# zhaihongjia/SplatLoc

Hardware: AMD Instinct MI355X
Metric: fwd+bwd frames/s @1080p, 500k Gaussians, 32 feat-ch; HBM GB/s vs roofline (higher is better)
Workload: dtype f32

## Files before the change

splatloc_amd/csrc/capi.hip:

```cpp
#include <string.h>

#include <mutex>
#include <unordered_map>
#include <string>
#include <vector>

#include "common.h"

namespace sr {

static thread_local std::string g_last_error;
static int g_deterministic = 0;
static int g_split_max_waves = SPLIT_MAX_WAVES;
void set_split_max_waves(int waves) { g_split_max_waves = waves < 0 ? SPLIT_MAX_WAVES : (waves > SPLIT_MAX_WAVES ? SPLIT_MAX_WAVES : waves); }
int split_max_waves() { return g_split_max_waves; }

void set_hip_error(hipError_t e, const char* what)
{
    g_last_error = std::string(what) + ": " + hipGetErrorString(e);
}

void set_error_text(const char* text) { g_last_error = text; }

struct StageRec { int stage; hipEvent_t a, b; };
// ... 129 lines not shown
    const size_t n = (size_t)(R > 0 ? R : 1);
    const size_t nv = (size_t)(V > 0 ? V : 1);
    const size_t tiles = (size_t)((W + TILE - 1) / TILE) * (size_t)((H + TILE - 1) / TILE) * nv;
    BinLayout L;
    size_t o = 0;
    auto take = [&](size_t bytes) { size_t at = o; o = align_up(o + bytes, 256); return at; };
    L.valsA = take(4 * n);
    L.keysA = take(4 * n);
    L.keysB = take(4 * n);
    L.valsB = take(4 * n);
    L.ranges = take(8 * (tiles > 0 ? tiles : 1));
    L.sort_tmp = take(sort_tmp_bytes((int64_t)n));
    L.irec = take(32 * n);
    L.ipack = take(4 * n);
    L.featp = take((C % 4) ? (size_t)(P > 0 ? P : 1) * padded_channels(C) * sizeof(float) : 16);
    L.gacc = take((size_t)(P > 0 ? P : 1) * nv * gacc_row_floats(C) * sizeof(float));
    L.pose_acc = take(POSE_ACC_BYTES);
    const bool ck = C <= 4 && 4 * (size_t)tiles <= (size_t)SPLIT_MAX_WAVES;
    L.ckpt = take(ck ? nv * (size_t)SPLIT_PARTS_MAX * (size_t)(C + 2) * (size_t)W * (size_t)H * sizeof(float) : 16);
    L.tile_order = take(4 * (tiles > 0 ? tiles : 1));
    L.nparts = take(4 * (tiles > 0 ? tiles : 1));
    L.bytes = o;
    return L;
}

BinView bin_view(void* base, int32_t P, int32_t V, int64_t R, int32_t W, int32_t H, int32_t C)
{
    const BinLayout L = bin_layout(P, V, R, W, H, C);
    char* b = reinterpret_cast<char*>(base);
    BinView v;
    v.point_list = reinterpret_cast<uint32_t*>(b + L.valsA);
// ... 17 lines not shown
{
    return align_up((size_t)W * H * 4 * (size_t)(V > 0 ? V : 1), 256);
}

ImgView img_view(void* base, int32_t W, int32_t H, int32_t V)
{
    char* b = reinterpret_cast<char*>(base);
    ImgView v;
    v.final_T = reinterpret_cast<float*>(b);
    v.n_contrib = reinterpret_cast<uint32_t*>(b + img_plane_bytes(W, H, V));
    return v;
}

static int check_row_index_range(int32_t P, int32_t V, int32_t C)
{
    const uint64_t row = (uint64_t)(gacc_row_floats(C) > padded_channels(C) ? gacc_row_floats(C) : padded_channels(C));
    const uint64_t n = (uint64_t)P * (uint64_t)V;
    if (n > (1ull << 24) || n * row >= (1ull << 32)) return SPLATRASTER_ERR_UNSUPPORTED;
    return SPLATRASTER_OK;
}

static int check_settings(const splatraster_settings* s)
{
    if (!s) return SPLATRASTER_ERR_BAD_ARG;
    if (s->image_width <= 0 || s->image_height <= 0 || s->channels <= 0) return SPLATRASTER_ERR_BAD_ARG;
    if (s->bg_channels < 0) return SPLATRASTER_ERR_BAD_ARG;
    return SPLATRASTER_OK;
}

}

using namespace sr;

// ... 358 lines not shown
        if (gcv != 0 && gcv < C) grads.gc = gcv;
    }
    for (int v = 0; v < V; ++v) {
        const int gcv = views[v].color_grad_channels ? views[v].color_grad_channels : C;
        if (gcv != grads.gc) return SPLATRASTER_ERR_BAD_ARG;
        grads.dL_dlast[v] = grads.gc < C ? views[v].dL_dout_last : nullptr;
    }
    for (int v = 0; v < V; ++v) {
        grads.out_color[v] = views[v].out_color;
        grads.out_depth[v] = views[v].out_depth;
        grads.dL_dcolor[v] = views[v].dL_dout_color;
        grads.dL_ddepth[v] = views[v].dL_dout_depth;
        grads.dL_dalpha[v] = views[v].dL_dout_alpha;
        grads.dL_dmeans2D[v] = views[v].dL_dmeans2D;
    }
    const size_t gacc_n = (size_t)gacc_row_floats(C) * (size_t)P * (size_t)V;
    const bool det = g_deterministic != 0;
    long long* gacc64 = nullptr;
    if (det) {
        SR_HIP_CHECK(hipMallocAsync(reinterpret_cast<void**>(&gacc64), sizeof(long long) * gacc_n, stream));
        SR_HIP_CHECK(hipMemsetAsync(gacc64, 0, sizeof(long long) * gacc_n, stream));
    }
    const bool pose = dL_dviewmatrix && dL_dprojmatrix;
    const size_t fill = pose ? (size_t)(reinterpret_cast<char*>(b.pose_acc) - reinterpret_cast<char*>(b.gacc)) + POSE_ACC_BYTES
                             : sizeof(float) * gacc_n;
    SR_HIP_CHECK(hipMemsetAsync(b.gacc, 0, fill, stream));
    grads.bg = bg;
    grads.bg_channels = bg ? s->bg_channels : 0;
    {
        StageTimer t(SPLATRASTER_STAGE_COMPOSITE_BWD, stream);
        if (det) st = launch_composite_bwd(*s, P, V, R, g, b, im, (C % 4) ? b.featp : feat, C, grads, b.gacc, gacc64, 0, stream);
        if (!st) st = launch_composite_bwd(*s, P, V, R, g, b, im, (C % 4) ? b.featp : feat, C, grads, b.gacc, gacc64, 1, stream);
    }
    if (det) {
        if (!st) st = launch_fixed_to_float((int64_t)gacc_n, gacc64, b.gacc, stream);
        (void)hipFreeAsync(gacc64, stream);
    }
    if (st) return st;
    StageTimer t(SPLATRASTER_STAGE_PREPROCESS_BWD, stream);
    return launch_preprocess_bwd(*s, P, V, cams, grads, means3D, shs, scales, rotations, cov3D_precomp, g.clamped, g.rec,
                                 b.gacc, C, shs ? nullptr : dL_dcolors, dL_dmeans3D, dL_dopacities,
                                 cov3D_precomp ? nullptr : dL_dscales, cov3D_precomp ? nullptr : dL_drotations,
                                 cov3D_precomp ? dL_dcov3D : nullptr, dL_dshs, dL_dviewmatrix, dL_dprojmatrix, dL_dcampos,
                                 b.pose_acc, stream, raw);
}

}

extern "C" {

// ... 542 lines not shown
```

splatloc_amd/csrc/common.h:

```cpp
#pragma once
#include <hip/hip_runtime.h>
#include <stdint.h>

#include "../../include/splatraster.h"

namespace sr {

constexpr int TILE = SPLATRASTER_TILE;
constexpr int TILE_PIX = TILE * TILE;
constexpr float NEAR_Z = 0.2f;
constexpr float DILATION = 0.3f;
constexpr float ALPHA_MAX = 0.99f;
constexpr float ALPHA_MIN = 1.0f / 255.0f;
constexpr float T_EPS = 0.0001f;
constexpr int WAVE = 64;
constexpr int PREPROCESS_BLOCK = 256;
static inline int preprocess_blocks(int32_t P) { return (P + PREPROCESS_BLOCK - 1) / PREPROCESS_BLOCK; }

void set_hip_error(hipError_t e, const char* what);
void set_error_text(const char* text);

int lookback_error_init();
int lookback_error_poll();
int lookback_set_spin_limit(uint32_t limit);
// ... 172 lines not shown
size_t bin_scratch_bytes(int32_t P, int32_t V, int tiles);
bool use_bins(int32_t P, int32_t V, int gx, int gy , size_t scratch_bytes);
int launch_bin_count(const splatraster_settings& s, int32_t P, int32_t V, const GeomView& g, uint32_t* table, void* scan_tmp,
                     hipStream_t stream);
int launch_bin_scatter_sort(const splatraster_settings& s, int32_t P, int32_t V, int64_t R, const GeomView& g,
                            const uint32_t* table, const BinView& b, uint64_t* keys, hipStream_t stream);

int launch_emit(const splatraster_settings& s, int32_t P, int32_t V, int64_t R, const GeomView& g, uint32_t* keys,
                uint32_t* vals, uint32_t* ranges, uint32_t nranges, hipStream_t stream);
int launch_ranges_clear(int32_t tiles, uint32_t* ranges, hipStream_t stream);
int launch_payload(const splatraster_settings& s, int32_t V, int64_t R, const GeomView& g, const BinView& b, hipStream_t stream);
int launch_pad_features(int32_t P, int C, const float* feat, float* featp, hipStream_t stream);
static inline int padded_channels(int C) { return (C + 3) & ~3; }
constexpr int POSE_SETS = 16, POSE_SET_FLOATS = 64;
constexpr size_t POSE_ACC_BYTES = (size_t)POSE_SETS * POSE_SET_FLOATS * sizeof(float) + 256;
__host__ __device__ static inline int gacc_moment_offset(int C) { return ((C & 15) + 7 <= 16) ? C : ((C + 15) & ~15); }
__host__ __device__ static inline int gacc_row_floats(int C) { return (gacc_moment_offset(C) + 7 + 15) & ~15; }
#ifndef SR_SPLIT_MAX_WAVES
#define SR_SPLIT_MAX_WAVES 6144
#endif
constexpr int SPLIT_MAX_WAVES = SR_SPLIT_MAX_WAVES;
constexpr int SPLIT_MIN_LIST = 256;
#ifndef SR_SPLIT_PARTS
#define SR_SPLIT_PARTS 4
#endif
constexpr int SPLIT_PARTS = SR_SPLIT_PARTS;
constexpr int SPLIT_PARTS_MAX = 4 * SPLIT_PARTS;
#ifndef SR_SPLIT_LONG
#define SR_SPLIT_LONG 1024
#endif
#ifndef SR_SPLIT_EXTRA_TILES
#define SR_SPLIT_EXTRA_TILES 512
// ... 20 lines not shown
                         const WinOut& out, hipStream_t stream);
#ifndef SR_TILE_ORDER
#define SR_TILE_ORDER 1
#endif
constexpr int TILE_ORDER_MAX_WAVES = 32768;
static inline bool use_tile_order(int V, int tiles_per_view) { return SR_TILE_ORDER && 4ll * V * tiles_per_view <= TILE_ORDER_MAX_WAVES; }
int launch_tile_order(const splatraster_settings& s, int32_t V, const BinView& b, hipStream_t stream);
int launch_composite_bwd(const splatraster_settings& s, int32_t P, int32_t V, int64_t R, const GeomView& g,
                         const BinView& b, const ImgView& im, const float* feat, int feat_stride,
                         const WinGrad& grads,
                         float* gacc ,
                         long long* gacc64 ,
                         int det_pass ,
                         hipStream_t stream);
void set_small_panel_max_waves(int waves);
int launch_fixed_to_float(int64_t n, const long long* src, float* dst, hipStream_t stream);

int launch_activate_fwd(int32_t P, int32_t K, int32_t deg, int32_t SC, int32_t E, const float* xyz,
                        const float* f_dc, const float* f_rest, const float* scaling, const float* rotation,
                        const float* opacity, const float* extra, const float* campos, float* scales,
                        float* rotations, float* opacities, float* colors, hipStream_t stream);
int launch_activate_bwd(int32_t P, int32_t K, int32_t deg, int32_t SC, int32_t E, const float* xyz,
                        const float* f_dc, const float* f_rest, const float* scaling, const float* rotation,
                        const float* opacity, const float* campos, const float* g_scales,
                        const float* g_rotations, const float* g_opacities, const float* g_colors, float* d_xyz,
                        float* d_f_dc, float* d_f_rest, float* d_scaling, float* d_rotation, float* d_opacity,
                        float* d_extra, hipStream_t stream);

struct StatsViews {
    const float* vs_grad[MAX_VIEWS];
    const int32_t* radii[MAX_VIEWS];
// ... 69 lines not shown
```

splatloc_amd/csrc/composite_bwd.hip:

```cpp
#include <type_traits>

#include "composite_common.h"

#ifndef SR_BWD_FS
#define SR_BWD_FS 32
#endif
#ifndef SR_BWD_STAGE_UNROLL
#define SR_BWD_STAGE_UNROLL 3
#endif

#ifndef SR_BWD_MINW
#define SR_BWD_MINW 4
#endif

#ifndef SR_BWD_DOT_CHAINS
#define SR_BWD_DOT_CHAINS 2
#endif
#ifndef SR_BWD_SMALL_PANEL_MAX_WAVES
#define SR_BWD_SMALL_PANEL_MAX_WAVES 6144
#endif
#ifndef SR_BWD_DOT_PREFETCH
#define SR_BWD_DOT_PREFETCH 1
#endif
#ifndef SR_BWD_TM
// ... 23 lines not shown
    static constexpr int ES = 9;
    static constexpr int KV = NV + ((XD || !AUX) ? 0 : 1) + (TM ? 0 : 6);
    static constexpr int NCP = (NC + 3) & ~3;
    static constexpr int FS = SR_BWD_FS;
    static constexpr int GROUP = 16;
    static constexpr int WS = 17;
};

constexpr int DET_HEADROOM_EXP = 170;
__device__ __forceinline__ int det_scale_exp(unsigned max_bits)
{
    const int eb = (int)((max_bits >> 23) & 0xffu);
    return DET_HEADROOM_EXP - (eb > 0 ? eb : 1);
}
template <bool DET>
__device__ __forceinline__ void acc_add(float* gacc, long long* gacc64, size_t idx, float v, int det_pass)
{
    if (DET) {
        if (det_pass == 0) {
            atomicMax(reinterpret_cast<unsigned*>(gacc) + idx, __float_as_uint(fabsf(v)));
        } else {
            const unsigned mb = __builtin_nontemporal_load(reinterpret_cast<const unsigned*>(gacc) + idx);
            if (((mb >> 23) & 0xffu) == 0xffu) {
                if (__builtin_isinf(v)) atomicAdd(reinterpret_cast<unsigned long long*>(gacc64) + idx, v > 0.f ? 1ull : (1ull << 32));
                return;
            }
            const double scaled = ldexp((double)v, det_scale_exp(mb));
            atomicAdd(reinterpret_cast<unsigned long long*>(gacc64) + idx, (unsigned long long)__double2ll_rn(scaled));
        }
    } else {
        (void)det_pass;
        atomicAdd(gacc + idx, v);
    }
}

template <int NC, bool SP, bool AUX>
constexpr int bwd_min_waves() { return (BwdCfg<NC, SP, AUX>::TM && NC >= 32) ? SR_BWD_MINW_TM : SR_BWD_MINW; }

template <int NC, bool DET, bool SP, bool AUX>
__global__ void __launch_bounds__(WAVE, (bwd_min_waves<NC, SP, AUX>()))
composite_bwd_kernel(int W, int H, int C_total, int CP4, int c0, int first_pass, int tiles , int V,
                     int P ,
                     const uint32_t* __restrict__ ranges, const uint32_t* __restrict__ ipack ,
                     const float4* __restrict__ irec, const float4* __restrict__ featp4,
                     WinGrad grads,
                     const float* __restrict__ final_T_all, const uint32_t* __restrict__ n_contrib_all,
                     float* __restrict__ gacc , int GROW,
                     int MO, long long* __restrict__ gacc64 ,
                     const float* __restrict__ ckpt_all ,
                     const uint32_t* __restrict__ nparts ,
                     int extra_blocks ,
                     const uint32_t* __restrict__ tile_order ,
                     int det_pass )
{
    using Cfg = BwdCfg<NC, SP, AUX>;
    using ST = typename std::conditional<DET, double, float>::type;
    constexpr int NCP = Cfg::NCP, NM = Cfg::NM, NV = Cfg::NV, KV = Cfg::KV, FS = Cfg::FS;
    constexpr int WS = Cfg::WS, GROUP = Cfg::GROUP;
    constexpr bool MFMA = Cfg::MFMA, XD = Cfg::XD;
    constexpr int NB = Cfg::NB;
    constexpr bool TM = Cfg::TM;
    constexpr int EG = Cfg::EG, ES = Cfg::ES;
    constexpr bool DOTM = NC >= SR_BWD_DOTM_MIN;
// ... 15 lines not shown
        const unsigned per = quadrant_blocks(SPLIT_EXTRA_TILES, gx);
        const unsigned group = blockIdx.x / per;
        int r;
        quadrant_of_block(blockIdx.x - group * per, SPLIT_EXTRA_TILES, gx, r, quad);
        if (r >= SPLIT_EXTRA_TILES || r >= V * tiles) return;
        gtile = (int)tile_order[r];
        seg_y += SPLIT_PARTS * (int)(group + 1u);
        if (seg_y >= (int)nparts[gtile]) return;
    } else {
        quadrant_of_block(blockIdx.x - (NC <= 4 ? (unsigned)extra_blocks : 0u), V * tiles, gx, gtile, quad, tile_order);
        if (gtile >= V * tiles) return;
    }
    const int view = (V == 1) ? 0 : gtile / tiles;
    const int tile = gtile - view * tiles;
    const uint32_t row0 = (uint32_t)view * (uint32_t)P;
    const float* __restrict__ dL_dcolor = grads.dL_dcolor[view];
    const float* __restrict__ dL_ddepth = grads.dL_ddepth[view];
    const float* __restrict__ dL_dalpha = grads.dL_dalpha[view];
    const float* __restrict__ dL_dlast = grads.dL_dlast[view];
    const int gc = grads.gc;
    const float* __restrict__ final_T = final_T_all + (size_t)view * H * W;
    const uint32_t* __restrict__ n_contrib = n_contrib_all + (size_t)view * H * W;
    const int lane = threadIdx.x;
    const int qx = (tile % gx) * TILE + (quad & 1) * 8, qy = (tile / gx) * TILE + (quad >> 1) * 8;
    const int px = qx + (lane & 7), py = qy + (lane >> 3);
    const bool inside = px < W && py < H;
    const float fx = (float)px, fy = (float)py;
    const size_t plane = (size_t)H * W;
    const size_t pix = inside ? (size_t)py * W + px : 0;
    uint32_t beg = ranges[2 * gtile], end0 = ranges[2 * gtile + 1];
// ... 75 lines not shown
            __builtin_amdgcn_wave_barrier();
#pragma unroll
            for (int ch = 0; ch < 16; ++ch) {
                const int c = 16 * t + ch;
                s_w[lane * WS + ch] = c < NC ? g[c < NC ? c : 0] : ((XD && c == NC) ? gD : 0.0f);
            }
            __builtin_amdgcn_wave_barrier();
#pragma unroll
            for (int kk = 0; kk < 16; ++kk) gt[kk][t] = s_w[(4 * kk + (lane >> 4)) * WS + (lane & 15)];
        }
        __builtin_amdgcn_wave_barrier();
    }
    uint32_t wave_last = last;
#pragma unroll
    for (int d = 1; d < WAVE; d <<= 1) wave_last = max(wave_last, (uint32_t)__shfl_xor((int)wave_last, d, WAVE));
    const uint32_t end = min(end0, list0 + wave_last);
    if (NC <= 4) { if (split && beg >= end) return; }

    const int slotv = (int)(__brev((unsigned)lane) >> 26);
    const bool slot_second = slotv >= KV;
    const int sv = slot_second ? slotv - KV : slotv;
    const bool slot_col = sv < NV;
    const bool slot_ok = slotv < 2 * KV;
    const int slot_off = slot_col ? (c0 + NM + sv) : (TM ? MO + 6 : MO + sv - NV);
    int nslot = 0;
    int e0 = 0;

    auto flush_panel = [&](int count) {
        __builtin_amdgcn_wave_barrier();
        f32x4 D[NB];
#pragma unroll
        for (int t = 0; t < NB; ++t) D[t] = f32x4{0.f, 0.f, 0.f, 0.f};
        const int row = (lane >> 4) * WS + (lane & 15);
#pragma unroll
        for (int kk = 0; kk < 16; ++kk) {
            const float a = s_w[4 * kk * WS + row];
#pragma unroll
            for (int t = 0; t < NB; ++t) {
                D[t] = __builtin_amdgcn_mfma_f32_16x16x4f32(a, gt[kk][t], D[t], 0, 0, 0);
            }
        }
        const int j0c = lane & 15;
#pragma unroll
        for (int r = 0; r < 4; ++r) {
            const int gs = 4 * (lane >> 4) + r;
            if (gs < count) {
                const uint32_t rowi = __umul24(s_gid[gs], (uint32_t)GROW);
#pragma unroll
                for (int t = 0; t < NB; ++t) {
                    const int c = 16 * t + j0c;
                    const bool full = 16 * t + 16 <= NM;
                    const bool col_ok = full || c < NM || (XD && c == NM && first_pass);
                    const uint32_t col_off = (full || c < NM) ? (uint32_t)(c0 + c) : (uint32_t)(MO + 6);
                    if (col_ok) acc_add<DET>(gacc, gacc64, (size_t)(rowi + col_off), D[t][r], det_pass);
                }
            }
        }
        __builtin_amdgcn_wave_barrier();
    };

    auto reduce_e = [&](int count) {
        if constexpr (TM) {
            __builtin_amdgcn_wave_barrier();
            const int eg = lane & 7, ei = lane >> 3;
            const float2 mu = s_emean[min(e0 + eg, GROUP - 1)];
            const float dx = mu.x - (float)(qx + ei);
            const float dy0 = mu.y - (float)qy;
            float m[6] = {0.f, 0.f, 0.f, 0.f, 0.f, 0.f};
#pragma unroll
            for (int j = 0; j < 8; ++j) {
                const float e = s_e[(8 * j + ei) * ES + eg];
                const float dy = dy0 - (float)j;
                const float ey = e * dy;
                m[5] += e;
                m[1] += ey;
                m[4] = fmaf(ey, dy, m[4]);
            }
            m[0] = m[5] * dx;
            m[2] = m[0] * dx;
            m[3] = m[1] * dx;
            const float outv = wave_reduce_hi3<6>(m, lane);
            const int vi = ((lane >> 5) & 1) + 2 * ((lane >> 4) & 1) + 4 * ((lane >> 3) & 1);
            if (eg < count && vi < 6) {
                const size_t di = (size_t)(__umul24(s_gid[e0 + eg], (uint32_t)GROW) + (uint32_t)(MO + vi));
                acc_add<DET>(gacc, gacc64, di, outv, det_pass);
            }
            __builtin_amdgcn_wave_barrier();
        }
    };

    uint32_t pw = 0;
    auto fetch = [&](uint32_t base, uint32_t& w_) {
        w_ = 0u;
        if (base + (uint32_t)lane < end) w_ = ipack[base + (uint32_t)lane];
    };
    if (beg >= end) return;
    const uint64_t gt_mask = (lane == WAVE - 1) ? 0ull : (~0ull << (lane + 1));
    const int nchunks = (int)((end - beg + (WAVE - 1)) / WAVE);
    fetch(beg + (uint32_t)(nchunks - 1) * WAVE, pw);

#pragma unroll 1
    for (int chunk = nchunks - 1; chunk >= 0; --chunk) {
        const uint32_t base = beg + (uint32_t)chunk * WAVE;
        const bool cur_reach = (pw >> (24 + quad)) & 1u;
        uint64_t cand = __builtin_amdgcn_ballot_w64(cur_reach);
        const uint32_t cur_gid = pw & 0xFFFFFFu;
        fetch(chunk > 0 ? base - WAVE : 0xFFFFFF00u, pw);
        const uint32_t idx0 = base - list0;
#pragma unroll 1
        while (cand != 0) {
            const int ncand = min(FS, (int)__popcll(cand));
            const int rank = __popcll(cand & gt_mask);
            const bool mine = cur_reach && ((cand >> lane) & 1ull) && rank < FS;
            __builtin_amdgcn_wave_barrier();
            if (mine) s_cgid[rank] = cur_gid;
            float4 rec_a = make_float4(0.f, 0.f, 0.f, 0.f), rec_b = rec_a;
            if (mine) {
                const size_t j = (size_t)base + lane;
                rec_a = irec[2 * j];
                rec_b = irec[2 * j + 1];
            }
            __builtin_amdgcn_wave_barrier();
#pragma unroll SR_BWD_STAGE_UNROLL
            for (int e = lane; e < ncand * PPR; e += WAVE) {
                const int row = e / PPR, pc = e - row * PPR;
                reinterpret_cast<float4*>(s_feat)[e] = featp4[(size_t)(__umul24(s_cgid[row] - row0, (uint32_t)CP4) + (uint32_t)((c0 >> 2) + pc))];
            }
            if (mine) {
                s_rec0[rank] = rec_a;
                s_rec1[rank] = rec_b;
            }
            __builtin_amdgcn_wave_barrier();
            auto process_pair = [&](int j0, int j1, bool has1, int r0, int r1, float qm0, float qm1) {
                const float4 p0 = s_rec0[r0], q0 = s_rec1[r0];
                const float4 p1 = s_rec0[r1], q1 = s_rec1[r1];
                const float dx0 = p0.x - fx, dy0 = p0.y - fy, dx1 = p1.x - fx, dy1 = p1.y - fy;
                const float pw0 = gauss_log2(q0, dx0, dy0), pw1 = gauss_log2(q1, dx1, dy1);
                const float Gr0 = exp2_core(pw0), Gr1 = exp2_core(pw1);
                const float ar0 = q0.w * Gr0, ar1 = q1.w * Gr1;
                const float al0 = fminf(ALPHA_MAX, ar0), al1 = fminf(ALPHA_MAX, ar1);
                const bool hit0 = (idx0 + (uint32_t)j0 < last) && pw0 <= 0.0f && ar0 >= ALPHA_MIN;
// ... 61 lines not shown
                        red[NV + 5] = E0;
                        red[KV + NV + 0] = Ex1;
                        red[KV + NV + 1] = Ey1;
                        red[KV + NV + 2] = Ex1 * dx1;
                        red[KV + NV + 3] = Ex1 * dy1;
                        red[KV + NV + 4] = Ey1 * dy1;
                        red[KV + NV + 5] = E1;
                    }
                    if constexpr (!XD && AUX) {
                        red[KV - 1] = w0 * gD;
                        red[2 * KV - 1] = w1 * gD;
                    }
                    {
                        const float outv = wave_reduce_pack<2 * KV>(red, lane);
                        const uint32_t gi = slot_second ? gi1 : gi0;
                        const size_t di = (size_t)(__umul24(gi, (uint32_t)GROW) + (uint32_t)slot_off);
                        if (slot_ok && (has1 || !slot_second)) acc_add<DET>(gacc, gacc64, di, outv, det_pass);
                    }
                }
                if constexpr (MFMA) {
                    s_w[lane * WS + nslot] = w0;
                    s_w[lane * WS + nslot + 1] = w1;
                    if constexpr (TM) {
                        s_e[lane * ES + (nslot - e0)] = E0;
                        s_e[lane * ES + (nslot - e0) + 1] = E1;
                    }
                    if (lane == 0) {
                        s_gid[nslot] = gi0;
                        s_gid[nslot + 1] = gi1;
                        if constexpr (TM) {
                            s_emean[nslot] = make_float2(p0.x, p0.y);
                            s_emean[nslot + 1] = make_float2(p1.x, p1.y);
// ... 82 lines not shown
    const WinGrad* grads;
    const float* ckpt;
    int det_pass;
};

template <int NC, bool DET, bool AUX = true>
static int launch_one_bwd(const splatraster_settings& s, int c0, int first, const GeomView& g,
                          const BinView& b, const ImgView& im, const float* feat, int feat_stride,
                          const BwdLaunch& L, float* gacc, long long* gacc64, hipStream_t stream)
{
    (void)g;
    const int gx = (s.image_width + TILE - 1) / TILE, gy = (s.image_height + TILE - 1) / TILE;
    const int tiles = gx * gy;
    const unsigned blocks = quadrant_blocks(L.V * tiles, gx);
    const float* ckpt = (NC <= 4 && c0 == 0 && first) ? L.ckpt : nullptr;
    const bool extras = ckpt != nullptr && use_tile_order(L.V, tiles);
    const unsigned extra_blocks = extras ? (unsigned)(SPLIT_PARTS_MAX / SPLIT_PARTS - 1) * quadrant_blocks(SPLIT_EXTRA_TILES, gx) : 0u;
    const dim3 grid(blocks + extra_blocks, ckpt ? (unsigned)SPLIT_PARTS : 1u);
#define SR_BWD_LAUNCH(SPV)                                                                                          \
    hipLaunchKernelGGL((composite_bwd_kernel<NC, DET, SPV, AUX>), grid, dim3(WAVE), 0, stream, s.image_width,           \
                       s.image_height, feat_stride, padded_channels(feat_stride) / 4, c0, first, tiles, L.V, L.P,      \
                       b.ranges, b.ipack, b.irec, reinterpret_cast<const float4*>(feat), *L.grads,       \
                       im.final_T, im.n_contrib, gacc, gacc_row_floats(s.channels),                                    \
                       gacc_moment_offset(s.channels), gacc64, ckpt, extras ? b.nparts : nullptr, (int)extra_blocks,               \
                       use_tile_order(L.V, tiles) ? b.tile_order : nullptr, L.det_pass)
    if constexpr (NC >= 4 && NC <= 15 && AUX) {
        if (4 * tiles <= g_small_panel_max_waves)
            SR_BWD_LAUNCH(true);
        else
            SR_BWD_LAUNCH(false);
    } else {
        SR_BWD_LAUNCH(false);
    }
#undef SR_BWD_LAUNCH
    SR_LAUNCH_CHECK();
    return SPLATRASTER_OK;
}

// ... 47 lines not shown
```

splatloc_amd/csrc/preprocess_bwd.hip:

```cpp
#include "composite_common.h"
#include "activation_math.h"

namespace sr {

__constant__ float BSH_C0 = 0.28209479177387814f;
__constant__ float BSH_C1 = 0.4886025119029199f;
__constant__ float BSH_C2[5] = {1.0925484305920792f, -1.0925484305920792f, 0.31539156525252005f,
                                -1.0925484305920792f, 0.5462742152960396f};
__constant__ float BSH_C3[7] = {-0.5900435899266435f, 2.890611442640554f, -0.4570457994644658f,
                                0.3731763325901154f,  -0.4570457994644658f, 1.445305721320277f,
                                -0.5900435899266435f};

__device__ void sh_backward(int deg, int M, const float* sh, float* dsh, const uint8_t* clamped,
                            const float* drgb_in, float ox, float oy, float oz, float* dmean)
{
    const float len = sqrtf(ox * ox + oy * oy + oz * oz);
    const float x = ox / len, y = oy / len, z = oz / len;
    float ddir[3] = {0.f, 0.f, 0.f};
    for (int ch = 0; ch < 3; ++ch) {
        const float d = clamped[ch] ? 0.f : drgb_in[ch];
        float ddx = 0.f, ddy = 0.f, ddz = 0.f;
#define SHV(k) sh[(k) * 3 + ch]
        dsh[0 * 3 + ch] = BSH_C0 * d;
        if (deg > 0) {
// ... 34 lines not shown
                }
            }
        }
#undef SHV
        for (int k = (deg + 1) * (deg + 1); k < M; ++k) dsh[k * 3 + ch] = 0.f;
        ddir[0] += ddx * d;
        ddir[1] += ddy * d;
        ddir[2] += ddz * d;
    }
    const float dot = x * ddir[0] + y * ddir[1] + z * ddir[2];
    dmean[0] += (ddir[0] - x * dot) / len;
    dmean[1] += (ddir[1] - y * dot) / len;
    dmean[2] += (ddir[2] - z * dot) / len;
}

template <bool POSE, bool RAW = false>
__global__ void __launch_bounds__(256)
preprocess_bwd_kernel(int P, int V, int W, int H, float mod, int sh_degree, int M, WinCams cams, WinGrad grads,
                      const float* __restrict__ means3D, const float* __restrict__ shs,
                      const float* __restrict__ scales, const float* __restrict__ rotations,
                      const float* __restrict__ cov3D_precomp,
                      const uint8_t* __restrict__ clamped,
                      const float4* __restrict__ rec, const float* __restrict__ gacc, int C, int GROW, int MO,
                      float* __restrict__ dL_dmeans3D,
                      float* __restrict__ dL_dopacities, float* __restrict__ dL_dscales,
                      float* __restrict__ dL_drotations, float* __restrict__ dL_dcov3D,
                      float* __restrict__ dL_dshs, float* __restrict__ dL_dview, float* __restrict__ dL_dproj,
                      float* __restrict__ dL_dcampos, float* __restrict__ pose_acc ,
                      RawBwd raw )
{
    const int i = blockIdx.x * blockDim.x + threadIdx.x;
    float pose[27];
#pragma unroll
    for (int k = 0; k < 27; ++k) pose[k] = 0.f;
    float dmean[3] = {0.f, 0.f, 0.f};
    float dscale[3] = {0.f, 0.f, 0.f};
    float drot[4] = {0.f, 0.f, 0.f, 0.f};
    float dcov[6] = {0.f, 0.f, 0.f, 0.f, 0.f, 0.f};
    float dop = 0.f;
    float csum[4] = {0.f, 0.f, 0.f, 0.f};
    if (i < P) {
    bool any_visible = false;
    const float px = means3D[3 * i], py = means3D[3 * i + 1], pz = means3D[3 * i + 2];
    float c6[6];
    float Rm[3][3] = {{0.f, 0.f, 0.f}, {0.f, 0.f, 0.f}, {0.f, 0.f, 0.f}}, sc[3] = {0.f, 0.f, 0.f};
    float4 qv = make_float4(0.f, 0.f, 0.f, 0.f);
    if (cov3D_precomp) {
#pragma unroll
        for (int k = 0; k < 6; ++k) c6[k] = cov3D_precomp[6 * i + k];
    } else {
        qv = reinterpret_cast<const float4*>(rotations)[i];
        const float r = qv.x, x = qv.y, y = qv.z, z = qv.w;
        Rm[0][0] = 1.f - 2.f * (y * y + z * z); Rm[0][1] = 2.f * (x * y - r * z); Rm[0][2] = 2.f * (x * z + r * y);
        Rm[1][0] = 2.f * (x * y + r * z); Rm[1][1] = 1.f - 2.f * (x * x + z * z); Rm[1][2] = 2.f * (y * z - r * x);
        Rm[2][0] = 2.f * (x * z - r * y); Rm[2][1] = 2.f * (y * z + r * x); Rm[2][2] = 1.f - 2.f * (x * x + y * y);
// ... 15 lines not shown

#pragma unroll 1
    for (int v = 0; v < V; ++v) {
    const float* __restrict__ view = cams.view[v];
    const float* __restrict__ proj = cams.proj[v];
    const float* __restrict__ campos_p = cams.campos[v];
    const float tanfovx = cams.tanfovx[v], tanfovy = cams.tanfovy[v];
    float Vm[16], PM[16];
#pragma unroll
    for (int k = 0; k < 16; ++k) { Vm[k] = view[k]; PM[k] = proj[k]; }
    const size_t gr = (size_t)v * P + i;
    float dm2x = 0.f, dm2y = 0.f;
    const bool visible = cams.radii[v][i] > 0;
    if (visible) {
        any_visible = true;
        const float* mrow = gacc + gr * GROW + MO;
        if constexpr (RAW) {
            const float4 cr = *reinterpret_cast<const float4*>(gacc + gr * GROW);
            csum[0] += cr.x; csum[1] += cr.y; csum[2] += cr.z; csum[3] += cr.w;
        }
        const float4 g0 = make_float4(mrow[0], mrow[1], mrow[2], mrow[3]);
        const float4 g1 = make_float4(mrow[4], mrow[5], mrow[6], 0.f);
        const float4 con = rec[2 * gr + 1];
        dm2x = -0.5f * (float)W * con.w * (con.x * g0.x + con.y * g0.y);
        dm2y = -0.5f * (float)H * con.w * (con.z * g0.y + con.y * g0.x);
        const float gA = -0.5f * con.w * g0.z, gB = -con.w * g0.w, gC = -0.5f * con.w * g1.x;
        dop += g1.y;
        const float gdepth = g1.z;
        const float tx0 = Vm[0] * px + Vm[4] * py + Vm[8] * pz + Vm[12];
        const float ty0 = Vm[1] * px + Vm[5] * py + Vm[9] * pz + Vm[13];
        const float tz = Vm[2] * px + Vm[6] * py + Vm[10] * pz + Vm[14];
        const float focal_x = (float)W / (2.0f * tanfovx), focal_y = (float)H / (2.0f * tanfovy);
        const float limx = 1.3f * tanfovx, limy = 1.3f * tanfovy;
        const float txtz = tx0 / tz, tytz = ty0 / tz;
// ... 81 lines not shown
        const float mul1 = hx * mw * mw, mul2 = hy * mw * mw;
        dmean[0] += (PM[0] * mw - PM[3] * mul1) * dm2x + (PM[1] * mw - PM[3] * mul2) * dm2y;
        dmean[1] += (PM[4] * mw - PM[7] * mul1) * dm2x + (PM[5] * mw - PM[7] * mul2) * dm2y;
        dmean[2] += (PM[8] * mw - PM[11] * mul1) * dm2x + (PM[9] * mw - PM[11] * mul2) * dm2y;
        if (POSE) {
            const float dh[3] = {dm2x * mw, dm2y * mw, -(mul1 * dm2x + mul2 * dm2y)};
            const float p4[4] = {px, py, pz, 1.f};
#pragma unroll
            for (int c = 0; c < 4; ++c)
#pragma unroll
                for (int j = 0; j < 3; ++j) pose[12 + 3 * c + j] = dh[j] * p4[c];
        }
        if (shs) {
            const float sm0 = dmean[0], sm1 = dmean[1], sm2 = dmean[2];
            sh_backward(sh_degree, M, shs + (size_t)i * 3 * M, dL_dshs + (size_t)i * 3 * M, clamped + 3 * (size_t)i,
                        gacc + gr * GROW, px - campos_p[0], py - campos_p[1], pz - campos_p[2], dmean);
            if (POSE) {
                pose[24] = -(dmean[0] - sm0);
                pose[25] = -(dmean[1] - sm1);
                pose[26] = -(dmean[2] - sm2);
            }
        }
    } else if (shs && dL_dshs) {
        for (int k = 0; k < 3 * M; ++k) dL_dshs[(size_t)i * 3 * M + k] = 0.f;
    }
    float* __restrict__ dm2 = grads.dL_dmeans2D[v];
    dm2[3 * i] = dm2x;
    dm2[3 * i + 1] = dm2y;
    dm2[3 * i + 2] = 0.f;
    }

// ... 57 lines not shown
            else if (e < 32) { const int j = (e - 16) & 3; if (j != 2) k = 12 + 3 * ((e - 16) >> 2) + (j == 3 ? 2 : j); }
            else k = 24 + (e - 32);
            float sum = 0.0f;
            if (k >= 0) {
                for (int q = 0; q < POSE_SETS; ++q)
                    sum += __hip_atomic_load(&pose_acc[q * POSE_SET_FLOATS + k], __ATOMIC_RELAXED, __HIP_MEMORY_SCOPE_AGENT);
            }
            if (e < 16) dL_dview[e] = sum;
            else if (e < 32) dL_dproj[e - 16] = sum;
            else if (dL_dcampos) dL_dcampos[e - 32] = sum;
        }
    }
    if (i < P) {
#pragma unroll
    for (int k = 0; k < 3; ++k) dL_dmeans3D[3 * i + k] = dmean[k];
    if constexpr (RAW) {
        if (raw.reg_row_grad) {
            const float o1 = raw.reg_out[1], rg = raw.reg_row_grad[i];
#pragma unroll
            for (int k = 0; k < 3; ++k) dscale[k] = act_add_scaled(dscale[k], raw.reg_weight, o1, rg);
        }
#pragma unroll
        for (int k = 0; k < 3; ++k) raw.d_scaling[3 * i + k] = dscale[k] * expf(raw.scaling[3 * (size_t)i + k]);
        reinterpret_cast<float4*>(raw.d_rotation)[i] =
            act_normalize_bwd(reinterpret_cast<const float4*>(raw.rotation)[i], make_float4(drot[0], drot[1], drot[2], drot[3]));
        raw.d_opacity[i] = act_sigmoid_bwd(dop, raw.opacity[i]);
#pragma unroll
        for (int c = 0; c < 3; ++c) {
            const float g = act_rgb_raw_deg0(raw.f_dc[3 * (size_t)i + c]) >= 0.0f ? csum[c] : 0.0f;
            raw.d_f_dc[3 * (size_t)i + c] = ACT_SH_C0 * g;
// ... 3 lines not shown
    }
    dL_dopacities[i] = dop;
    if (dL_dscales) {
#pragma unroll
        for (int k = 0; k < 3; ++k) dL_dscales[3 * i + k] = dscale[k];
    }
    if (dL_drotations) reinterpret_cast<float4*>(dL_drotations)[i] = make_float4(drot[0], drot[1], drot[2], drot[3]);
    if (dL_dcov3D) {
#pragma unroll
        for (int k = 0; k < 6; ++k) dL_dcov3D[6 * i + k] = dcov[k];
    }
    }
}

__global__ void __launch_bounds__(256)
fixed_to_float_kernel(int64_t n, const long long* __restrict__ src, float* __restrict__ dst)
{
    const int64_t e = (int64_t)blockIdx.x * blockDim.x + threadIdx.x;
    if (e >= n) return;
    const unsigned mb = reinterpret_cast<const unsigned*>(dst)[e];
    const int eb = (int)((mb >> 23) & 0xffu);
    if (eb == 255) {
        const unsigned long long cnt = (unsigned long long)src[e];
        const bool pos = (cnt & 0xffffffffull) != 0, neg = (cnt >> 32) != 0;
        dst[e] = ((mb & 0x7fffffu) || pos == neg) ? __builtin_nanf("") : (neg ? -__builtin_inff() : __builtin_inff());
        return;
    }
    dst[e] = (float)ldexp((double)src[e], -(170 - (eb > 0 ? eb : 1)));
}

int launch_fixed_to_float(int64_t n, const long long* src, float* dst, hipStream_t stream)
{
    if (n <= 0) return SPLATRASTER_OK;
    hipLaunchKernelGGL(fixed_to_float_kernel, dim3((unsigned)((n + 255) / 256)), dim3(256), 0, stream, n, src, dst);
    SR_LAUNCH_CHECK();
    return SPLATRASTER_OK;
}

__global__ void __launch_bounds__(256)
gather_dcolors_kernel(int64_t n, int C, int GROW, int V, int64_t P, const float* __restrict__ gacc,
                      float* __restrict__ dL_dcolors)
{
    const int64_t e = (int64_t)blockIdx.x * blockDim.x + threadIdx.x;
    if (e >= n) return;
    const int64_t i = e / C;
    const int ch = (int)(e - i * C);
    float sum = gacc[i * GROW + ch];
    for (int v = 1; v < V; ++v) sum += gacc[(v * P + i) * GROW + ch];
    dL_dcolors[e] = sum;
}

int launch_preprocess_bwd(const splatraster_settings& s, int32_t P, int32_t V, const WinCams& cams, const WinGrad& grads,
                          const float* means3D, const float* shs, const float* scales, const float* rotations,
                          const float* cov3D_precomp, const uint8_t* clamped, const float4* rec, const float* gacc, int C,
                          float* dL_dcolors, float* dL_dmeans3D, float* dL_dopacities, float* dL_dscales,
                          float* dL_drotations, float* dL_dcov3D, float* dL_dshs, float* dL_dview,
                          float* dL_dproj, float* dL_dcampos, float* pose_acc, hipStream_t stream, const RawBwd* raw)
{
    if (P == 0) return SPLATRASTER_OK;
    if (dL_dcolors && !raw) {
        const int64_t n = (int64_t)P * C;
        hipLaunchKernelGGL(gather_dcolors_kernel, dim3((unsigned)((n + 255) / 256)), dim3(256), 0, stream, n, C,
                           gacc_row_floats(C), V, (int64_t)P, gacc, dL_dcolors);
        SR_LAUNCH_CHECK();
    }
    const bool pose = dL_dview && dL_dproj;
    if (pose && !pose_acc) return SPLATRASTER_ERR_BAD_ARG;
#define SR_PBWD_ARGS                                                                                              \
    P, V, s.image_width, s.image_height, s.scale_modifier, s.sh_degree, s.sh_coeffs, cams, grads, means3D,         \
        shs, scales, rotations, cov3D_precomp, clamped, rec, gacc, C, gacc_row_floats(C),                          \
        gacc_moment_offset(C), dL_dmeans3D, dL_dopacities, dL_dscales, dL_drotations,                              \
        dL_dcov3D, dL_dshs, dL_dview, dL_dproj, dL_dcampos, pose_acc, (raw ? *raw : RawBwd{})
    if (raw) {
        if (pose || shs || cov3D_precomp || !scales || !rotations || raw->E > 1) return SPLATRASTER_ERR_UNSUPPORTED;
        hipLaunchKernelGGL((preprocess_bwd_kernel<false, true>), dim3((P + 255) / 256), dim3(256), 0, stream, SR_PBWD_ARGS);
    } else if (pose)
        hipLaunchKernelGGL(preprocess_bwd_kernel<true>, dim3((P + 255) / 256), dim3(256), 0, stream, SR_PBWD_ARGS);
    else
        hipLaunchKernelGGL(preprocess_bwd_kernel<false>, dim3((P + 255) / 256), dim3(256), 0, stream, SR_PBWD_ARGS);
#undef SR_PBWD_ARGS
    SR_LAUNCH_CHECK();
    return SPLATRASTER_OK;
}

}
```

Baseline: 737.2.

## Split gradient accumulator into shared color table plus per-view tail rows

Restructures the gradient accumulation buffer so the first multiple-of-16 color channels (for C>=32) live in one table shared across views, and only the remaining channels and moments stay per-view. This shrinks the memset and accumulator footprint and replaces the per-view color gather with a direct copy, with the tail colors summed inside the preprocess backward kernel. It adds a layout struct and index math in the hot kernels, specialises the C=35 case with constants, and reduces fixed-point headroom in deterministic mode to absorb cross-view summation into shared slots. Atomic contention on shared columns may rise when there are several views.

```diff
diff --git a/splatloc_amd/csrc/capi.hip b/splatloc_amd/csrc/capi.hip
--- a/splatloc_amd/csrc/capi.hip
+++ b/splatloc_amd/csrc/capi.hip
@@ -167,7 +167,7 @@
     L.irec = take(32 * n);
     L.ipack = take(4 * n);
     L.featp = take((C % 4) ? (size_t)(P > 0 ? P : 1) * padded_channels(C) * sizeof(float) : 16);
-    L.gacc = take((size_t)(P > 0 ? P : 1) * nv * gacc_row_floats(C) * sizeof(float));
+    L.gacc = take(gacc_total_floats(C, (size_t)(P > 0 ? P : 1), nv) * sizeof(float));
     L.pose_acc = take(POSE_ACC_BYTES);
     const bool ck = C <= 4 && 4 * (size_t)tiles <= (size_t)SPLIT_MAX_WAVES;
     L.ckpt = take(ck ? nv * (size_t)SPLIT_PARTS_MAX * (size_t)(C + 2) * (size_t)W * (size_t)H * sizeof(float) : 16);
@@ -215,9 +215,9 @@
 
 static int check_row_index_range(int32_t P, int32_t V, int32_t C)
 {
-    const uint64_t row = (uint64_t)(gacc_row_floats(C) > padded_channels(C) ? gacc_row_floats(C) : padded_channels(C));
     const uint64_t n = (uint64_t)P * (uint64_t)V;
-    if (n > (1ull << 24) || n * row >= (1ull << 32)) return SPLATRASTER_ERR_UNSUPPORTED;
+    if (n > (1ull << 24) || n * (uint64_t)padded_channels(C) >= (1ull << 32)) return SPLATRASTER_ERR_UNSUPPORTED;
+    if ((uint64_t)gacc_total_floats(C, (size_t)P, (size_t)V) >= (1ull << 32)) return SPLATRASTER_ERR_UNSUPPORTED;
     return SPLATRASTER_OK;
 }
 
@@ -606,7 +606,7 @@
         grads.dL_dalpha[v] = views[v].dL_dout_alpha;
         grads.dL_dmeans2D[v] = views[v].dL_dmeans2D;
     }
-    const size_t gacc_n = (size_t)gacc_row_floats(C) * (size_t)P * (size_t)V;
+    const size_t gacc_n = gacc_total_floats(C, (size_t)P, (size_t)V);
     const bool det = g_deterministic != 0;
     long long* gacc64 = nullptr;
     if (det) {
@@ -625,7 +625,7 @@
         if (!st) st = launch_composite_bwd(*s, P, V, R, g, b, im, (C % 4) ? b.featp : feat, C, grads, b.gacc, gacc64, 1, stream);
     }
     if (det) {
-        if (!st) st = launch_fixed_to_float((int64_t)gacc_n, gacc64, b.gacc, stream);
+        if (!st) st = launch_fixed_to_float((int64_t)gacc_n, gacc64, b.gacc, gacc_det_headroom_drop(C, V), stream);
         (void)hipFreeAsync(gacc64, stream);
     }
     if (st) return st;
diff --git a/splatloc_amd/csrc/common.h b/splatloc_amd/csrc/common.h
--- a/splatloc_amd/csrc/common.h
+++ b/splatloc_amd/csrc/common.h
@@ -210,8 +210,30 @@
 static inline int padded_channels(int C) { return (C + 3) & ~3; }
 constexpr int POSE_SETS = 16, POSE_SET_FLOATS = 64;
 constexpr size_t POSE_ACC_BYTES = (size_t)POSE_SETS * POSE_SET_FLOATS * sizeof(float) + 256;
-__host__ __device__ static inline int gacc_moment_offset(int C) { return ((C & 15) + 7 <= 16) ? C : ((C + 15) & ~15); }
-__host__ __device__ static inline int gacc_row_floats(int C) { return (gacc_moment_offset(C) + 7 + 15) & ~15; }
+__host__ __device__ constexpr int gacc_moment_offset(int C) { return ((C & 15) + 7 <= 16) ? C : ((C + 15) & ~15); }
+__host__ __device__ constexpr int gacc_row_floats(int C) { return (gacc_moment_offset(C) + 7 + 15) & ~15; }
+__host__ __device__ constexpr int gacc_shared_floats(int C) { return C >= 32 ? (C & ~15) : 0; }
+__host__ __device__ constexpr int gacc_view_floats(int C) { return gacc_row_floats(C) - gacc_shared_floats(C); }
+__host__ __device__ static inline size_t gacc_total_floats(int C, size_t P, size_t V)
+{
+    return P * (size_t)gacc_shared_floats(C) + V * P * (size_t)gacc_view_floats(C);
+}
+struct GaccLayout {
+    uint32_t SH, PV;
+    uint32_t P;
+    __host__ __device__ size_t index(size_t g, size_t i, uint32_t col) const
+    {
+        return col < SH ? i * SH + col : (size_t)P * SH + g * PV + (col - SH);
+    }
+    __host__ __device__ uint32_t view_base24(uint32_t row0) const { return P * SH + row0 * PV - SH; }
+    __host__ __device__ uint32_t stride24(uint32_t col) const { return col < SH ? SH : PV; }
+    __host__ __device__ uint32_t base24(uint32_t col, uint32_t row0) const { return col < SH ? 0u : view_base24(row0); }
+};
+__host__ __device__ constexpr int gacc_det_headroom_drop(int C, int V) { return (gacc_shared_floats(C) > 0 && V > 1) ? 3 : 0; }
+__host__ __device__ static inline GaccLayout gacc_layout(int C, int32_t P)
+{
+    return GaccLayout{(uint32_t)gacc_shared_floats(C), (uint32_t)gacc_view_floats(C), (uint32_t)P};
+}
 #ifndef SR_SPLIT_MAX_WAVES
 #define SR_SPLIT_MAX_WAVES 6144
 #endif
@@ -262,7 +284,7 @@
                          int det_pass ,
                          hipStream_t stream);
 void set_small_panel_max_waves(int waves);
-int launch_fixed_to_float(int64_t n, const long long* src, float* dst, hipStream_t stream);
+int launch_fixed_to_float(int64_t n, const long long* src, float* dst, int headroom_drop , hipStream_t stream);
 
 int launch_activate_fwd(int32_t P, int32_t K, int32_t deg, int32_t SC, int32_t E, const float* xyz,
                         const float* f_dc, const float* f_rest, const float* scaling, const float* rotation,
diff --git a/splatloc_amd/csrc/composite_bwd.hip b/splatloc_amd/csrc/composite_bwd.hip
--- a/splatloc_amd/csrc/composite_bwd.hip
+++ b/splatloc_amd/csrc/composite_bwd.hip
@@ -61,7 +61,7 @@
     return DET_HEADROOM_EXP - (eb > 0 ? eb : 1);
 }
 template <bool DET>
-__device__ __forceinline__ void acc_add(float* gacc, long long* gacc64, size_t idx, float v, int det_pass)
+__device__ __forceinline__ void acc_add(float* gacc, long long* gacc64, size_t idx, float v, int det_pass, int det_drop)
 {
     if (DET) {
         if (det_pass == 0) {
@@ -72,11 +72,12 @@
                 if (__builtin_isinf(v)) atomicAdd(reinterpret_cast<unsigned long long*>(gacc64) + idx, v > 0.f ? 1ull : (1ull << 32));
                 return;
             }
-            const double scaled = ldexp((double)v, det_scale_exp(mb));
+            const double scaled = ldexp((double)v, det_scale_exp(mb) - det_drop);
             atomicAdd(reinterpret_cast<unsigned long long*>(gacc64) + idx, (unsigned long long)__double2ll_rn(scaled));
         }
     } else {
         (void)det_pass;
+        (void)det_drop;
         atomicAdd(gacc + idx, v);
     }
 }
@@ -92,8 +93,8 @@
                      const float4* __restrict__ irec, const float4* __restrict__ featp4,
                      WinGrad grads,
                      const float* __restrict__ final_T_all, const uint32_t* __restrict__ n_contrib_all,
-                     float* __restrict__ gacc , int GROW,
-                     int MO, long long* __restrict__ gacc64 ,
+                     float* __restrict__ gacc , GaccLayout GL,
+                     int MO , long long* __restrict__ gacc64 ,
                      const float* __restrict__ ckpt_all ,
                      const uint32_t* __restrict__ nparts ,
                      int extra_blocks ,
@@ -139,6 +140,14 @@
     const int view = (V == 1) ? 0 : gtile / tiles;
     const int tile = gtile - view * tiles;
     const uint32_t row0 = (uint32_t)view * (uint32_t)P;
+    constexpr bool WIDE = NC >= 32;
+    const int det_drop = DET ? gacc_det_headroom_drop(C_total, V) : 0;
+    static_assert(!WIDE || (Cfg::NM == 32 && NC < 48), "a wide kernel's flush columns are the shared table's, its butterfly columns the per-view row's");
+    constexpr bool FIXED = NC == 35;
+    static_assert(!FIXED || (gacc_shared_floats(NC) == 32 && gacc_view_floats(NC) == 16 && gacc_shared_floats(NC + 1) == 32 &&
+                             gacc_view_floats(NC + 1) == 16), "the constants of the headline kernel");
+    if constexpr (FIXED) { GL.SH = 32u; GL.PV = 16u; }
+    const uint32_t pv_base = GL.view_base24(row0);
     const float* __restrict__ dL_dcolor = grads.dL_dcolor[view];
     const float* __restrict__ dL_ddepth = grads.dL_ddepth[view];
     const float* __restrict__ dL_dalpha = grads.dL_dalpha[view];
@@ -244,7 +253,8 @@
     uint32_t wave_last = last;
 #pragma unroll
     for (int d = 1; d < WAVE; d <<= 1) wave_last = max(wave_last, (uint32_t)__shfl_xor((int)wave_last, d, WAVE));
-    const uint32_t end = min(end0, list0 + wave_last);
+    uint32_t end = min(end0, list0 + wave_last);
+    if constexpr (WIDE) end = (uint32_t)__builtin_amdgcn_readfirstlane((int)end);
     if (NC <= 4) { if (split && beg >= end) return; }
 
     const int slotv = (int)(__brev((unsigned)lane) >> 26);
@@ -252,7 +262,9 @@
     const int sv = slot_second ? slotv - KV : slotv;
     const bool slot_col = sv < NV;
     const bool slot_ok = slotv < 2 * KV;
-    const int slot_off = slot_col ? (c0 + NM + sv) : (TM ? MO + 6 : MO + sv - NV);
+    const uint32_t slot_colv = (uint32_t)(slot_col ? (c0 + NM + sv) : (TM ? MO + 6 : MO + sv - NV));
+    const uint32_t slot_stride = WIDE ? GL.PV : GL.stride24(slot_colv);
+    const uint32_t slot_off = (WIDE ? pv_base : GL.base24(slot_colv, row0)) + slot_colv;
     int nslot = 0;
     int e0 = 0;
 
@@ -275,14 +287,15 @@
         for (int r = 0; r < 4; ++r) {
             const int gs = 4 * (lane >> 4) + r;
             if (gs < count) {
-                const uint32_t rowi = __umul24(s_gid[gs], (uint32_t)GROW);
+                const uint32_t gid = s_gid[gs];
 #pragma unroll
                 for (int t = 0; t < NB; ++t) {
                     const int c = 16 * t + j0c;
                     const bool full = 16 * t + 16 <= NM;
                     const bool col_ok = full || c < NM || (XD && c == NM && first_pass);
-                    const uint32_t col_off = (full || c < NM) ? (uint32_t)(c0 + c) : (uint32_t)(MO + 6);
-                    if (col_ok) acc_add<DET>(gacc, gacc64, (size_t)(rowi + col_off), D[t][r], det_pass);
+                    const uint32_t col = (full || c < NM) ? (uint32_t)(c0 + c) : (uint32_t)(MO + 6);
+                    const uint32_t rowi = WIDE ? __umul24(gid, GL.SH) : __umul24(gid, GL.stride24(col)) + GL.base24(col, row0);
+                    if (col_ok) acc_add<DET>(gacc, gacc64, (size_t)(rowi + col), D[t][r], det_pass, det_drop);
                 }
             }
         }
@@ -312,8 +325,8 @@
             const float outv = wave_reduce_hi3<6>(m, lane);
             const int vi = ((lane >> 5) & 1) + 2 * ((lane >> 4) & 1) + 4 * ((lane >> 3) & 1);
             if (eg < count && vi < 6) {
-                const size_t di = (size_t)(__umul24(s_gid[e0 + eg], (uint32_t)GROW) + (uint32_t)(MO + vi));
-                acc_add<DET>(gacc, gacc64, di, outv, det_pass);
+                const size_t di = (size_t)(__umul24(s_gid[e0 + eg], GL.PV) + pv_base + (uint32_t)(MO + vi));
+                acc_add<DET>(gacc, gacc64, di, outv, det_pass, det_drop);
             }
             __builtin_amdgcn_wave_barrier();
         }
@@ -334,7 +347,7 @@
         const uint32_t base = beg + (uint32_t)chunk * WAVE;
         const bool cur_reach = (pw >> (24 + quad)) & 1u;
         uint64_t cand = __builtin_amdgcn_ballot_w64(cur_reach);
-        const uint32_t cur_gid = pw & 0xFFFFFFu;
+        const uint32_t cur_gid = (pw & 0xFFFFFFu) - row0;
         fetch(chunk > 0 ? base - WAVE : 0xFFFFFF00u, pw);
         const uint32_t idx0 = base - list0;
 #pragma unroll 1
@@ -354,7 +367,7 @@
 #pragma unroll SR_BWD_STAGE_UNROLL
             for (int e = lane; e < ncand * PPR; e += WAVE) {
                 const int row = e / PPR, pc = e - row * PPR;
-                reinterpret_cast<float4*>(s_feat)[e] = featp4[(size_t)(__umul24(s_cgid[row] - row0, (uint32_t)CP4) + (uint32_t)((c0 >> 2) + pc))];
+                reinterpret_cast<float4*>(s_feat)[e] = featp4[(size_t)(__umul24(s_cgid[row], (uint32_t)CP4) + (uint32_t)((c0 >> 2) + pc))];
             }
             if (mine) {
                 s_rec0[rank] = rec_a;
@@ -446,8 +459,8 @@
                     {
                         const float outv = wave_reduce_pack<2 * KV>(red, lane);
                         const uint32_t gi = slot_second ? gi1 : gi0;
-                        const size_t di = (size_t)(__umul24(gi, (uint32_t)GROW) + (uint32_t)slot_off);
-                        if (slot_ok && (has1 || !slot_second)) acc_add<DET>(gacc, gacc64, di, outv, det_pass);
+                        const size_t di = (size_t)(__umul24(gi, slot_stride) + slot_off);
+                        if (slot_ok && (has1 || !slot_second)) acc_add<DET>(gacc, gacc64, di, outv, det_pass, det_drop);
                     }
                 }
                 if constexpr (MFMA) {
@@ -560,6 +573,8 @@
     const int tiles = gx * gy;
     const unsigned blocks = quadrant_blocks(L.V * tiles, gx);
     const float* ckpt = (NC <= 4 && c0 == 0 && first) ? L.ckpt : nullptr;
+    const GaccLayout GL = gacc_layout(s.channels, L.P);
+    if (NC == 35 && (c0 != 0 || GL.SH != 32u || GL.PV != 16u)) return SPLATRASTER_ERR_UNSUPPORTED;
     const bool extras = ckpt != nullptr && use_tile_order(L.V, tiles);
     const unsigned extra_blocks = extras ? (unsigned)(SPLIT_PARTS_MAX / SPLIT_PARTS - 1) * quadrant_blocks(SPLIT_EXTRA_TILES, gx) : 0u;
     const dim3 grid(blocks + extra_blocks, ckpt ? (unsigned)SPLIT_PARTS : 1u);
@@ -567,7 +582,7 @@
     hipLaunchKernelGGL((composite_bwd_kernel<NC, DET, SPV, AUX>), grid, dim3(WAVE), 0, stream, s.image_width,           \
                        s.image_height, feat_stride, padded_channels(feat_stride) / 4, c0, first, tiles, L.V, L.P,      \
                        b.ranges, b.ipack, b.irec, reinterpret_cast<const float4*>(feat), *L.grads,       \
-                       im.final_T, im.n_contrib, gacc, gacc_row_floats(s.channels),                                    \
+                       im.final_T, im.n_contrib, gacc, GL,                                                             \
                        gacc_moment_offset(s.channels), gacc64, ckpt, extras ? b.nparts : nullptr, (int)extra_blocks,               \
                        use_tile_order(L.V, tiles) ? b.tile_order : nullptr, L.det_pass)
     if constexpr (NC >= 4 && NC <= 15 && AUX) {
diff --git a/splatloc_amd/csrc/preprocess_bwd.hip b/splatloc_amd/csrc/preprocess_bwd.hip
--- a/splatloc_amd/csrc/preprocess_bwd.hip
+++ b/splatloc_amd/csrc/preprocess_bwd.hip
@@ -72,15 +72,15 @@
     dmean[2] += (ddir[2] - z * dot) / len;
 }
 
-template <bool POSE, bool RAW = false>
+template <bool POSE, bool RAW = false, int TQ = 0>
 __global__ void __launch_bounds__(256)
 preprocess_bwd_kernel(int P, int V, int W, int H, float mod, int sh_degree, int M, WinCams cams, WinGrad grads,
                       const float* __restrict__ means3D, const float* __restrict__ shs,
                       const float* __restrict__ scales, const float* __restrict__ rotations,
                       const float* __restrict__ cov3D_precomp,
                       const uint8_t* __restrict__ clamped,
-                      const float4* __restrict__ rec, const float* __restrict__ gacc, int C, int GROW, int MO,
-                      float* __restrict__ dL_dmeans3D,
+                      const float4* __restrict__ rec, const float* __restrict__ gacc, int C, GaccLayout GL, int MO,
+                      float* __restrict__ dL_dcolors , float* __restrict__ dL_dmeans3D,
                       float* __restrict__ dL_dopacities, float* __restrict__ dL_dscales,
                       float* __restrict__ dL_drotations, float* __restrict__ dL_dcov3D,
                       float* __restrict__ dL_dshs, float* __restrict__ dL_dview, float* __restrict__ dL_dproj,
@@ -97,6 +97,11 @@
     float dcov[6] = {0.f, 0.f, 0.f, 0.f, 0.f, 0.f};
     float dop = 0.f;
     float csum[4] = {0.f, 0.f, 0.f, 0.f};
+    constexpr int NT = TQ > 0 ? 4 * TQ : 1;
+    float tsum[NT];
+#pragma unroll
+    for (int k = 0; k < NT; ++k) tsum[k] = 0.f;
+    [[maybe_unused]] const int ntail = C - (int)GL.SH;
     if (i < P) {
     bool any_visible = false;
     const float px = means3D[3 * i], py = means3D[3 * i + 1], pz = means3D[3 * i + 2];
@@ -142,10 +147,18 @@
     const bool visible = cams.radii[v][i] > 0;
     if (visible) {
         any_visible = true;
-        const float* mrow = gacc + gr * GROW + MO;
+        const float* mrow = gacc + GL.index(gr, (size_t)i, (uint32_t)MO);
         if constexpr (RAW) {
-            const float4 cr = *reinterpret_cast<const float4*>(gacc + gr * GROW);
+            const float4 cr = *reinterpret_cast<const float4*>(gacc + GL.index(gr, (size_t)i, 0u));
             csum[0] += cr.x; csum[1] += cr.y; csum[2] += cr.z; csum[3] += cr.w;
+        }
+        if constexpr (TQ > 0) {
+            const float4* trow = reinterpret_cast<const float4*>(gacc + GL.index(gr, (size_t)i, GL.SH));
+#pragma unroll
+            for (int q = 0; q < TQ; ++q) {
+                const float4 t = trow[q];
+                tsum[4 * q] += t.x; tsum[4 * q + 1] += t.y; tsum[4 * q + 2] += t.z; tsum[4 * q + 3] += t.w;
+            }
         }
         const float4 g0 = make_float4(mrow[0], mrow[1], mrow[2], mrow[3]);
         const float4 g1 = make_float4(mrow[4], mrow[5], mrow[6], 0.f);
@@ -257,7 +270,7 @@
         if (shs) {
             const float sm0 = dmean[0], sm1 = dmean[1], sm2 = dmean[2];
             sh_backward(sh_degree, M, shs + (size_t)i * 3 * M, dL_dshs + (size_t)i * 3 * M, clamped + 3 * (size_t)i,
-                        gacc + gr * GROW, px - campos_p[0], py - campos_p[1], pz - campos_p[2], dmean);
+                        gacc + GL.index(gr, (size_t)i, 0u), px - campos_p[0], py - campos_p[1], pz - campos_p[2], dmean);
             if (POSE) {
                 pose[24] = -(dmean[0] - sm0);
                 pose[25] = -(dmean[1] - sm1);
@@ -345,6 +358,11 @@
     if (i < P) {
 #pragma unroll
     for (int k = 0; k < 3; ++k) dL_dmeans3D[3 * i + k] = dmean[k];
+    if constexpr (TQ > 0) {
+#pragma unroll
+        for (int k = 0; k < NT; ++k)
+            if (k < ntail) dL_dcolors[(size_t)i * C + GL.SH + k] = tsum[k];
+    }
     if constexpr (RAW) {
         if (raw.reg_row_grad) {
             const float o1 = raw.reg_out[1], rg = raw.reg_row_grad[i];
@@ -378,7 +396,7 @@
 }
 
 __global__ void __launch_bounds__(256)
-fixed_to_float_kernel(int64_t n, const long long* __restrict__ src, float* __restrict__ dst)
+fixed_to_float_kernel(int64_t n, const long long* __restrict__ src, float* __restrict__ dst, int headroom_drop)
 {
     const int64_t e = (int64_t)blockIdx.x * blockDim.x + threadIdx.x;
     if (e >= n) return;
@@ -390,28 +408,37 @@
         dst[e] = ((mb & 0x7fffffu) || pos == neg) ? __builtin_nanf("") : (neg ? -__builtin_inff() : __builtin_inff());
         return;
     }
-    dst[e] = (float)ldexp((double)src[e], -(170 - (eb > 0 ? eb : 1)));
-}
-
-int launch_fixed_to_float(int64_t n, const long long* src, float* dst, hipStream_t stream)
+    dst[e] = (float)ldexp((double)src[e], -(170 - headroom_drop - (eb > 0 ? eb : 1)));
+}
+
+int launch_fixed_to_float(int64_t n, const long long* src, float* dst, int headroom_drop, hipStream_t stream)
 {
     if (n <= 0) return SPLATRASTER_OK;
-    hipLaunchKernelGGL(fixed_to_float_kernel, dim3((unsigned)((n + 255) / 256)), dim3(256), 0, stream, n, src, dst);
+    hipLaunchKernelGGL(fixed_to_float_kernel, dim3((unsigned)((n + 255) / 256)), dim3(256), 0, stream, n, src, dst, headroom_drop);
     SR_LAUNCH_CHECK();
     return SPLATRASTER_OK;
 }
 
 __global__ void __launch_bounds__(256)
-gather_dcolors_kernel(int64_t n, int C, int GROW, int V, int64_t P, const float* __restrict__ gacc,
+gather_dcolors_kernel(int64_t n, int C, GaccLayout GL, int V, const float* __restrict__ gacc,
                       float* __restrict__ dL_dcolors)
 {
     const int64_t e = (int64_t)blockIdx.x * blockDim.x + threadIdx.x;
     if (e >= n) return;
     const int64_t i = e / C;
     const int ch = (int)(e - i * C);
-    float sum = gacc[i * GROW + ch];
-    for (int v = 1; v < V; ++v) sum += gacc[(v * P + i) * GROW + ch];
+    float sum = gacc[GL.index((size_t)i, (size_t)i, (uint32_t)ch)];
+    for (int v = 1; v < V; ++v) sum += gacc[GL.index((size_t)v * GL.P + (size_t)i, (size_t)i, (uint32_t)ch)];
     dL_dcolors[e] = sum;
+}
+__global__ void __launch_bounds__(256)
+copy_shared_dcolors_kernel(int64_t n , int C, GaccLayout GL, const float* __restrict__ gacc, float* __restrict__ dL_dcolors)
+{
+    const int64_t e = (int64_t)blockIdx.x * blockDim.x + threadIdx.x;
+    if (e >= n) return;
+    const int64_t i = e / GL.SH;
+    const uint32_t ch = (uint32_t)(e - i * GL.SH);
+    dL_dcolors[i * C + ch] = gacc[GL.index((size_t)i, (size_t)i, ch)];
 }
 
 int launch_preprocess_bwd(const splatraster_settings& s, int32_t P, int32_t V, const WinCams& cams, const WinGrad& grads,
@@ -422,26 +449,37 @@
                           float* dL_dproj, float* dL_dcampos, float* pose_acc, hipStream_t stream, const RawBwd* raw)
 {
     if (P == 0) return SPLATRASTER_OK;
+    const GaccLayout GL = gacc_layout(C, P);
+    const int ntail = (dL_dcolors && !raw && GL.SH > 0) ? C - (int)GL.SH : 0;
     if (dL_dcolors && !raw) {
-        const int64_t n = (int64_t)P * C;
-        hipLaunchKernelGGL(gather_dcolors_kernel, dim3((unsigned)((n + 255) / 256)), dim3(256), 0, stream, n, C,
-                           gacc_row_floats(C), V, (int64_t)P, gacc, dL_dcolors);
+        const int64_t n = (int64_t)P * (GL.SH ? (int)GL.SH : C);
+        if (GL.SH)
+            hipLaunchKernelGGL(copy_shared_dcolors_kernel, dim3((unsigned)((n + 255) / 256)), dim3(256), 0, stream, n, C, GL, gacc,
+                               dL_dcolors);
+        else
+            hipLaunchKernelGGL(gather_dcolors_kernel, dim3((unsigned)((n + 255) / 256)), dim3(256), 0, stream, n, C, GL, V, gacc,
+                               dL_dcolors);
         SR_LAUNCH_CHECK();
     }
     const bool pose = dL_dview && dL_dproj;
     if (pose && !pose_acc) return SPLATRASTER_ERR_BAD_ARG;
 #define SR_PBWD_ARGS                                                                                              \
     P, V, s.image_width, s.image_height, s.scale_modifier, s.sh_degree, s.sh_coeffs, cams, grads, means3D,         \
-        shs, scales, rotations, cov3D_precomp, clamped, rec, gacc, C, gacc_row_floats(C),                          \
-        gacc_moment_offset(C), dL_dmeans3D, dL_dopacities, dL_dscales, dL_drotations,                              \
+        shs, scales, rotations, cov3D_precomp, clamped, rec, gacc, C, GL,                                          \
+        gacc_moment_offset(C), dL_dcolors, dL_dmeans3D, dL_dopacities, dL_dscales, dL_drotations,                              \
         dL_dcov3D, dL_dshs, dL_dview, dL_dproj, dL_dcampos, pose_acc, (raw ? *raw : RawBwd{})
     if (raw) {
         if (pose || shs || cov3D_precomp || !scales || !rotations || raw->E > 1) return SPLATRASTER_ERR_UNSUPPORTED;
         hipLaunchKernelGGL((preprocess_bwd_kernel<false, true>), dim3((P + 255) / 256), dim3(256), 0, stream, SR_PBWD_ARGS);
-    } else if (pose)
-        hipLaunchKernelGGL(preprocess_bwd_kernel<true>, dim3((P + 255) / 256), dim3(256), 0, stream, SR_PBWD_ARGS);
-    else
-        hipLaunchKernelGGL(preprocess_bwd_kernel<false>, dim3((P + 255) / 256), dim3(256), 0, stream, SR_PBWD_ARGS);
+    } else if (pose) {
+        if (ntail > 4) hipLaunchKernelGGL((preprocess_bwd_kernel<true, false, 4>), dim3((P + 255) / 256), dim3(256), 0, stream, SR_PBWD_ARGS);
+        else if (ntail > 0) hipLaunchKernelGGL((preprocess_bwd_kernel<true, false, 1>), dim3((P + 255) / 256), dim3(256), 0, stream, SR_PBWD_ARGS);
+        else hipLaunchKernelGGL(preprocess_bwd_kernel<true>, dim3((P + 255) / 256), dim3(256), 0, stream, SR_PBWD_ARGS);
+    } else {
+        if (ntail > 4) hipLaunchKernelGGL((preprocess_bwd_kernel<false, false, 4>), dim3((P + 255) / 256), dim3(256), 0, stream, SR_PBWD_ARGS);
+        else if (ntail > 0) hipLaunchKernelGGL((preprocess_bwd_kernel<false, false, 1>), dim3((P + 255) / 256), dim3(256), 0, stream, SR_PBWD_ARGS);
+        else hipLaunchKernelGGL(preprocess_bwd_kernel<false>, dim3((P + 255) / 256), dim3(256), 0, stream, SR_PBWD_ARGS);
+    }
 #undef SR_PBWD_ARGS
     SR_LAUNCH_CHECK();
     return SPLATRASTER_OK;
```

After: 752.9, median of 6. 2.1% higher.
